# Xiaoming-Zhao/PointNav-VO

Hardware: AMD Instinct MI355X
Metric: RGB-D frame-pair VO inferences/s @341x192 (higher is better)
Workload: dtype f32

## Files before the change

### pointnav-vo_amd/csrc/conv_x3.hip

```cpp
#include <cmath>
#include <cstdio>
#include <cstdlib>
#include <cstring>

#include "pnvo_internal.h"

namespace pnvo {

typedef float f32x16 __attribute__((ext_vector_type(16)));
typedef float f32x4 __attribute__((ext_vector_type(4)));
typedef float f32x2 __attribute__((ext_vector_type(2)));
typedef __bf16 bf16x8 __attribute__((ext_vector_type(8)));
typedef __bf16 bf16x2 __attribute__((ext_vector_type(2)));
typedef _Float16 f16x8 __attribute__((ext_vector_type(8)));
typedef _Float16 f16x2 __attribute__((ext_vector_type(2)));
typedef unsigned u32x4 __attribute__((ext_vector_type(4)));

namespace {
__device__ __forceinline__ unsigned pack2(float a, float b) {
  const bf16x2 r = __builtin_convertvector(f32x2{a, b}, bf16x2);
  return __builtin_bit_cast(unsigned, r);
}
__device__ __forceinline__ unsigned pack2h(float a, float b) {
  const f16x2 r = __builtin_convertvector(f32x2{a, b}, f16x2);
  return __builtin_bit_cast(unsigned, r);
}
__device__ __forceinline__ float lo_f(unsigned u) { return __builtin_bit_cast(float, u << 16); }
__device__ __forceinline__ float hi_f(unsigned u) { return __builtin_bit_cast(float, u & 0xffff0000u); }
}

constexpr int x3_wpe(int mw, int nw, int np, bool dsf = false) {
  return dsf ? (mw * nw >= 6 ? 1 : (mw * nw >= 2 ? 2 : 3)) : ((np == 2 && mw * nw <= 2) ? 3 : 2);
}

template <int KS, int STRIDE, int MODE, int MW, int NW, int NP, bool DSF = false, bool W8 = false, bool KSW = false, bool M16 = false>
__global__ __launch_bounds__(W8 ? 512 : 256) __attribute__((amdgpu_waves_per_eu(W8 ? 2 : x3_wpe(MW, NW, NP, DSF), W8 ? 2 : x3_wpe(MW, NW, NP, DSF)))) void conv_x3_kernel(const ConvX3Args p) {
  constexpr int NTH = W8 ? 512 : 256, NWV = NTH / 64;
  constexpr int EMW = KSW ? 1 : MW;
  constexpr int NWT = M16 ? NW / 2 : NW;
  constexpr int TW = M16 ? (MW * NW + 3) / 4 : MW * NW;
  static_assert(!M16 || (NP == 2 && KS == 3 && STRIDE == 1 && !DSF && !KSW && NW % 2 == 0), "16x16x32 flavour: float16-piece 3x3 stride-1 convs, whole N-tiles");
  static_assert(!KSW || (NW == 1 && NP == 2 && KS == 3 && !DSF && !W8), "K split over the waves: float16-piece 3x3 convs, one N-tile");
  static_assert(!DSF || (KS == 3 && STRIDE == 2 && NP == 2 && (MODE == 0 || MODE == 2)), "the downsample rides on a float16-piece 3x3 stride-2 conv");
  extern __shared__ __attribute__((aligned(16))) unsigned char lds[];
  constexpr int PSTEP = KS == 1 ? STRIDE : 1;
  constexpr int CS = KS == 1 ? 1 : STRIDE;
  constexpr int PAD = KS / 2;
  const int lane = threadIdx.x & 63;
  const int wave = __builtin_amdgcn_readfirstlane(threadIdx.x >> 6);

  const int ntiles = p.B * p.tiles_r * p.tiles_c;
  const int chunk = (ntiles + 7) >> 3;
  int bid = (int)(blockIdx.x & 7) * chunk + (int)(blockIdx.x >> 3);
  if (bid >= ntiles) return;
  const int tci = bid % p.tiles_c;
  bid /= p.tiles_c;
  const int tri = bid % p.tiles_r;
  const int n = bid / p.tiles_r;
  const int r0 = tri * p.TR, c0 = tci * p.TC;
  const int hi0 = r0 * STRIDE - PAD, wi0 = c0 * STRIDE - PAD;
  const int mdl = (p.grp_end0 > 0 && n >= p.grp_end0) + (p.grp_end1 > 0 && n >= p.grp_end1);
  const unsigned short *g_wpk = mdl == 0 ? p.wpk : p.wpk_g[mdl - 1];
  const unsigned short *g_ds_wpk = mdl == 0 ? p.ds_wpk : p.ds_wpk_g[mdl - 1];
  const float g_oscale = mdl == 0 ? p.oscale : p.oscale_g[mdl - 1], g_ds_oscale = mdl == 0 ? p.ds_oscale : p.ds_oscale_g[mdl - 1];
  const float *g_gamma = mdl == 0 ? p.gn_gamma : p.gn_gamma_g[mdl - 1], *g_beta = mdl == 0 ? p.gn_beta : p.gn_beta_g[mdl - 1];
  const float *g_ds_gamma = mdl == 0 ? p.ds_gamma : p.ds_gamma_g[mdl - 1], *g_ds_beta = mdl == 0 ? p.ds_beta : p.ds_beta_g[mdl - 1];
  const int PR = p.PR, PC = p.PC, CK = p.CK;
  const int pitch = CK * 2 + 16;
  const int plane = PR * PC * pitch;
  const int npix = p.TR * p.TC;
  const int tab_off = KSW ? max(NP * plane, 4 * MW * 4096) : NP * plane;
  unsigned *qtab = reinterpret_cast<unsigned *>(lds + tab_off);
  unsigned *otab = qtab + p.MT * 32;
  for (int e = (int)threadIdx.x; e < p.MT * 32; e += NTH) {
    const int q = min(e, npix - 1);
    const int tr = q / p.TC, tc = q - tr * p.TC;
    qtab[e] = (unsigned)(((tr * CS) * PC + tc * CS) * pitch);
    const bool ok = e < npix && r0 + tr < p.Ho && c0 + tc < p.Wo;
    otab[e] = (unsigned)((tr * p.Wo + tc) * p.COUTP) | (ok ? 0u : 0x80000000u);
  }

  const int wn = p.wn;
  const int wave_m = wave / wn;
  const int wave_n = (wave & (wn - 1)) + (int)blockIdx.y * wn;
  const int ntt = p.COUTP >> 5, kct = p.CIN >> 4;

  f32x16 acc[MW][NW];
#pragma unroll
  for (int i = 0; i < MW; ++i)
#pragma unroll
    for (int j = 0; j < NW; ++j)
#pragma unroll
      for (int r = 0; r < 16; ++r) acc[i][j][r] = 0.f;
  f32x4 acc16[M16 ? MW : 1][M16 ? NW : 1];
  const int mt16 = (npix + 15) >> 4;
  const int m16_row = (mt16 + NWV / wn - 1) / (NWV / wn), m16_sub0 = wave_m * m16_row;
  const bool m16_last = m16_sub0 + MW <= mt16 && MW <= m16_row;
  if (M16) {
#pragma unroll
    for (int i = 0; i < MW; ++i)
#pragma unroll
      for (int j = 0; j < NW; ++j) acc16[M16 ? i : 0][M16 ? j : 0] = f32x4{0.f, 0.f, 0.f, 0.f};
  }
  f32x16 accd[DSF ? MW : 1][DSF ? NW : 1];
  if (DSF) {
#pragma unroll
    for (int i = 0; i < MW; ++i)
#pragma unroll
      for (int j = 0; j < NW; ++j)
#pragma unroll
        for (int r = 0; r < 16; ++r) accd[DSF ? i : 0][DSF ? j : 0][r] = 0.f;
  }

  float in_mul = 1.f, in_div = 1.f;
  const bool in_scaled = NP == 2 && p.in_absmax != nullptr;
  if (in_scaled) {
    unsigned mb = p.in_absmax[(threadIdx.x & 63) * 16];
#pragma unroll
    for (int d = 32; d >= 1; d >>= 1) mb = max(mb, (unsigned)__shfl_xor((int)mb, d));
    const int e = mb != 0u ? (int)((mb >> 23) & 0xffu) - 126 : 14;
    in_mul = __builtin_bit_cast(float, (unsigned)(14 - e + 127) << 23);
    in_div = __builtin_bit_cast(float, (unsigned)(e - 14 + 127) << 23);
  }
  const int G = CK >> 3;
  const int cg = threadIdx.x & (G - 1), pl = threadIdx.x / G, PS = NTH / G;
  const int dr = PS / PC, dc = PS - dr * PC;
  const int nppix = PR * PC;

  unsigned long long c_stage = 0, c_mm = 0, t_0 = __builtin_readcyclecounter(), r_0 = wall_clock64();
  for (int ck0 = 0; ck0 < p.CIN; ck0 += CK) {
    unsigned long long t_a = __builtin_readcyclecounter();
    if (ck0 > 0) __syncthreads();
    {
      f32x4 sc0, sc1, sh0, sh1, rs0, rs1, rt0, rt1;
      const bool res_ss = MODE == 2 && p.res_scale != nullptr;
      auto load_ss = [&]() {
        if (MODE >= 1) {
          const float *ps = p.in_scale + (long)n * p.CIN + ck0 + 8 * cg;
          const float *pt = p.in_shift + (long)n * p.CIN + ck0 + 8 * cg;
          sc0 = *reinterpret_cast<const f32x4 *>(ps);
          sc1 = *reinterpret_cast<const f32x4 *>(ps + 4);
          sh0 = *reinterpret_cast<const f32x4 *>(pt);
          sh1 = *reinterpret_cast<const f32x4 *>(pt + 4);
        }
        if (res_ss) {
          const float *ps = p.res_scale + (long)n * p.CIN + ck0 + 8 * cg;
          const float *pt = p.res_shift + (long)n * p.CIN + ck0 + 8 * cg;
          rs0 = *reinterpret_cast<const f32x4 *>(ps);
          rs1 = *reinterpret_cast<const f32x4 *>(ps + 4);
          rt0 = *reinterpret_cast<const f32x4 *>(pt);
          rt1 = *reinterpret_cast<const f32x4 *>(pt + 4);
        }
      };
      load_ss();
      int pr = pl / PC, pc = pl - pr * PC;
      const long img = ((long)n * p.H * p.W) * p.CIN + ck0 + 8 * cg;
      const float *xb = p.x + img;
      struct Round {
        f32x4 v[2][2], w[2][2];
        unsigned off[2];
        int gofs[2];
        bool ok[2], in[2], own[2];
      };
      auto fetch = [&](int pix, Round &r) {
#pragma unroll
        for (int k = 0; k < 2; ++k) {
          const int hi = hi0 + pr * PSTEP, wi = wi0 + pc * PSTEP;
          r.ok[k] = pix + k * PS < nppix;
          r.in[k] = r.ok[k] && hi >= 0 && hi < p.H && wi >= 0 && wi < p.W;
          r.off[k] = (unsigned)((pr * PC + pc) * pitch + 16 * cg);
          r.v[k][0] = r.v[k][1] = f32x4{0.f, 0.f, 0.f, 0.f};
          if (MODE >= 2) {
            r.own[k] = r.in[k] && p.xout != nullptr && blockIdx.y == 0 && pr >= PAD && pr < PAD + p.TR * CS && pc >= PAD && pc < PAD + p.TC * CS;
            r.gofs[k] = (hi * p.W + wi) * p.CIN;
          }
          if (r.in[k]) {
            const float *src = xb + ((long)hi * p.W + wi) * p.CIN;
            r.v[k][0] = *reinterpret_cast<const f32x4 *>(src);
            r.v[k][1] = *reinterpret_cast<const f32x4 *>(src + 4);
            if (MODE == 2) {
              const float *rsrc = p.res + img + ((long)hi * p.W + wi) * p.CIN;
              r.w[k][0] = *reinterpret_cast<const f32x4 *>(rsrc);
              r.w[k][1] = *reinterpret_cast<const f32x4 *>(rsrc + 4);
            }
          }
          pr += dr;
          pc += dc;
          if (pc >= PC) {
            pc -= PC;
            pr += 1;
          }
        }
      };
      auto split_store = [&](const Round &r) {
#pragma unroll
        for (int k = 0; k < 2; ++k) {
          if (!r.ok[k]) continue;
          float f[8];
#pragma unroll
          for (int e = 0; e < 8; ++e) {
            float t = r.v[k][e >> 2][e & 3];
            if (MODE == 1) {
              const f32x4 &sc = e < 4 ? sc0 : sc1, &sh = e < 4 ? sh0 : sh1;
              t = r.in[k] ? fmaxf(__builtin_fmaf(t, sc[e & 3], sh[e & 3]), 0.f) : 0.f;
            }
            if (MODE == 3) {
              const f32x4 &sc = e < 4 ? sc0 : sc1, &sh = e < 4 ? sh0 : sh1;
              int key = __builtin_bit_cast(int, t);
              key = key >= 0 ? key : key ^ 0x7fffffff;
              t = r.in[k] ? fmaxf(__builtin_fmaf(__builtin_bit_cast(float, key), __builtin_fabsf(sc[e & 3]), sh[e & 3]), 0.f) : 0.f;
            }
            if (MODE == 2) {
              const f32x4 &sc = e < 4 ? sc0 : sc1, &sh = e < 4 ? sh0 : sh1;
              float u = r.w[k][e >> 2][e & 3];
              if (res_ss) u = __builtin_fmaf(u, (e < 4 ? rs0 : rs1)[e & 3], (e < 4 ? rt0 : rt1)[e & 3]);
              t = r.in[k] ? fmaxf(__builtin_fmaf(t, sc[e & 3], sh[e & 3]) + u, 0.f) : 0.f;
            }
            f[e] = t;
          }
          if (MODE >= 2 && r.own[k]) {
            float *dst = p.xout + img + r.gofs[k];
            *reinterpret_cast<f32x4 *>(dst) = f32x4{f[0], f[1], f[2], f[3]};
            *reinterpret_cast<f32x4 *>(dst + 4) = f32x4{f[4], f[5], f[6], f[7]};
          }
          if (NP == 2) {
            if (in_scaled) {
#pragma unroll
              for (int e = 0; e < 8; ++e) f[e] *= in_mul;
            }
            u32x4 o0, o1;
#pragma unroll
            for (int e = 0; e < 4; ++e) {
              const float a = f[2 * e], b = f[2 * e + 1];
              const f16x2 h = __builtin_convertvector(f32x2{a, b}, f16x2);
              o0[e] = __builtin_bit_cast(unsigned, h);
              o1[e] = pack2h(a - (float)h[0], b - (float)h[1]);
            }
            *reinterpret_cast<u32x4 *>(lds + r.off[k]) = o0;
            *reinterpret_cast<u32x4 *>(lds + plane + r.off[k]) = o1;
            continue;
          }
          u32x4 o0, o1, o2;
#pragma unroll
          for (int e = 0; e < 4; ++e) {
            const float a = f[2 * e], b = f[2 * e + 1];
            const unsigned h = pack2(a, b);
            const float ra = a - lo_f(h), rb = b - hi_f(h);
            const unsigned m = pack2(ra, rb);
            o0[e] = h;
            o1[e] = m;
            o2[e] = pack2(ra - lo_f(m), rb - hi_f(m));
          }
          *reinterpret_cast<u32x4 *>(lds + r.off[k]) = o0;
          *reinterpret_cast<u32x4 *>(lds + plane + r.off[k]) = o1;
          *reinterpret_cast<u32x4 *>(lds + 2 * plane + r.off[k]) = o2;
        }
      };
      constexpr bool PIPE = !((MODE == 2 && (TW >= 6 || (M16 && !W8) || x3_wpe(MW, NW, NP) == 3 || DSF)) || (DSF && MW * NW == 4));
      if (TW <= 2 && !(MODE == 2 && (x3_wpe(MW, NW, NP) == 3 || DSF))) {
        for (int pix = pl; pix < nppix; pix += 6 * PS) {
          Round r0, r1, r2;
          fetch(pix, r0);
          fetch(pix + 2 * PS, r1);
          fetch(pix + 4 * PS, r2);
          split_store(r0);
          split_store(r1);
          split_store(r2);
        }
      } else if (PIPE) {
        Round cur, nxt;
        fetch(pl, cur);
        for (int pix = pl; pix < nppix; pix += 2 * PS) {
          const bool more = pix + 2 * PS < nppix;
          if (more) fetch(pix + 2 * PS, nxt);
          split_store(cur);
          if (more) cur = nxt;
        }
      } else {
        for (int pix = pl; pix < nppix; pix += 2 * PS) {
          Round cur;
          fetch(pix, cur);
          split_store(cur);
        }
      }
    }
    __syncthreads();
    unsigned long long t_b = __builtin_readcyclecounter();
    c_stage += t_b - t_a;

    if constexpr (M16) {
      unsigned aoff[MW];
#pragma unroll
      for (int i = 0; i < MW; ++i) {
        const int sub = min(m16_sub0 + i, mt16 - 1);
        aoff[i] = qtab[sub * 16 + (lane & 15)] + (unsigned)((lane >> 4) * 16);
      }
      const int kcc = CK >> 4, kcp = CK >> 5;
      const int nsteps = KS * KS * kcp;
      const unsigned kstep = (unsigned)ntt * (NP * 1024u);
      const char *wb_n = reinterpret_cast<const char *>(g_wpk) + (long)(ck0 >> 4) * kstep;
      unsigned toff_n = 0;
      int kc_n = 0, kw_n = 0;
      auto advance = [&]() {
        ++kc_n;
        toff_n += 64;
        wb_n += 2 * kstep;
        if (kc_n == kcp) {
          kc_n = 0;
          toff_n += (unsigned)(pitch - kcp * 64);
          wb_n += (long)(kct - kcc) * kstep;
          if (++kw_n == KS) {
            kw_n = 0;
            toff_n += (unsigned)((PC - KS) * pitch);
          }
        }
      };
      const int kg = lane >> 4;
      unsigned voff[NW];
#pragma unroll
      for (int j = 0; j < NW; ++j)
        voff[j] = (unsigned)min(wave_n * NWT + (j >> 1), ntt - 1) * (NP * 1024u) + (unsigned)(kg >> 1) * kstep +
                  (unsigned)((kg & 1) * 32 + 16 * (j & 1) + (lane & 15)) * 16u;
      auto loadA = [&](int i, u32x4 (*a)[MW]) {
#pragma unroll
        for (int pc = 0; pc < NP; ++pc) a[pc][i] = *reinterpret_cast<const u32x4 *>(lds + pc * plane + aoff[i] + toff_n);
      };
      auto loadB = [&](u32x4 (*b)[NW]) {
#pragma unroll
        for (int j = 0; j < NW; ++j)
#pragma unroll
          for (int pc = 0; pc < NP; ++pc) b[pc][j] = *reinterpret_cast<const u32x4 *>(wb_n + (size_t)voff[j] + pc * 1024);
      };
      auto step = [&](u32x4 (*a)[MW], const u32x4 (*b)[NW]) {
#pragma unroll
        for (int i = 0; i < MW; ++i) {
          if (i == MW - 1 && !m16_last) break;
          constexpr int TA[3] = {1, 0, 0}, TB[3] = {0, 1, 0};
#pragma unroll
          for (int jt = 0; jt < NWT; ++jt)
#pragma unroll
            for (int t = 0; t < 3; ++t)
#pragma unroll
              for (int j = 2 * jt; j < 2 * jt + 2; ++j)
                acc16[M16 ? i : 0][M16 ? j : 0] = __builtin_amdgcn_mfma_f32_16x16x32_f16(__builtin_bit_cast(f16x8, a[TA[t]][i]), __builtin_bit_cast(f16x8, b[TB[t]][M16 ? j : 0]),
                                                                                         acc16[M16 ? i : 0][M16 ? j : 0], 0, 0, 0);
          __builtin_amdgcn_sched_barrier(0);
          loadA(i, a);
          __builtin_amdgcn_sched_barrier(0);
        }
      };
      u32x4 a[NP][MW], b0[NP][NW], b1[NP][NW];
      loadB(b0);
#pragma unroll
      for (int i = 0; i < MW; ++i) loadA(i, a);
      advance();
#pragma unroll 1
      for (int s = 0; s < nsteps; s += 2) {
        loadB(b1);
        __builtin_amdgcn_sched_barrier(0);
        step(a, b0);
        if (s + 2 < nsteps) advance();
        if (s + 1 < nsteps) {
          loadB(b0);
          __builtin_amdgcn_sched_barrier(0);
          step(a, b1);
          if (s + 3 < nsteps) advance();
        }
      }
    } else {
    unsigned aoff[MW];
#pragma unroll
    for (int i = 0; i < MW; ++i) {
      const int mt = min(KSW ? i : wave_m * MW + i, p.MT - 1);
      aoff[i] = qtab[mt * 32 + (lane & 31)] + (unsigned)((lane >> 5) * 16);
    }
    const int kcc = CK >> 4;
    const int nsteps = KS * KS * kcc;
    const unsigned kstep = (unsigned)ntt * (NP * 1024u);
    const char *wb_n = reinterpret_cast<const char *>(g_wpk) + (long)(ck0 >> 4) * kstep;
    unsigned toff_n = 0;
    int kc_n = 0, kw_n = 0;
    auto advance = [&]() {
      ++kc_n;
      toff_n += 32;
      wb_n += kstep;
      if (kc_n == kcc) {
        kc_n = 0;
        toff_n += (unsigned)(pitch - kcc * 32);
        wb_n += (long)(kct - kcc) * kstep;
        if (++kw_n == KS) {
          kw_n = 0;
          toff_n += (unsigned)((PC - KS) * pitch);
        }
      }
    };
    constexpr bool RING = NP == 2 && KS == 3 && MW * NW <= 2;
    const char *wb_b = wb_n;
    int kc_b = 0;
    auto advanceB = [&]() {
      wb_b += kstep;
      if (++kc_b == kcc) {
        kc_b = 0;
        wb_b += (long)(kct - kcc) * kstep;
      }
    };
    unsigned voff[NW];
#pragma unroll
    for (int j = 0; j < NW; ++j) voff[j] = (unsigned)min(wave_n * NW + j, ntt - 1) * (NP * 1024u) + (unsigned)lane * 16u;
    auto loadBr = [&](u32x4 (*b)[NW]) {
#pragma unroll
      for (int j = 0; j < NW; ++j)
#pragma unroll
        for (int pc = 0; pc < NP; ++pc) b[pc][j] = *reinterpret_cast<const u32x4 *>(wb_b + (size_t)voff[j] + pc * 1024);
    };
    auto loadA = [&](int i, u32x4 (*a)[MW]) {
#pragma unroll
      for (int pc = 0; pc < NP; ++pc) a[pc][i] = *reinterpret_cast<const u32x4 *>(lds + pc * plane + aoff[i] + toff_n);
    };
    auto loadB = [&](u32x4 (*b)[NW]) {
#pragma unroll
      for (int j = 0; j < NW; ++j)
#pragma unroll
        for (int pc = 0; pc < NP; ++pc) b[pc][j] = *reinterpret_cast<const u32x4 *>(wb_n + (size_t)voff[j] + pc * 1024);
    };
    auto step = [&](u32x4 (*a)[MW], const u32x4 (*b)[NW]) {
#pragma unroll
      for (int i = 0; i < MW; ++i) {
#pragma unroll
        for (int j = 0; j < NW; ++j) {
          if (NP == 2) {
            constexpr int TA[3] = {1, 0, 0}, TB[3] = {0, 1, 0};
#pragma unroll
            for (int t = 0; t < 3; ++t)
              acc[i][j] = __builtin_amdgcn_mfma_f32_32x32x16_f16(__builtin_bit_cast(f16x8, a[TA[t]][i]),
                                                                 __builtin_bit_cast(f16x8, b[TB[t]][j]), acc[i][j], 0, 0, 0);
          } else {
            constexpr int TA[6] = {1, 2, 0, 1, 0, 0}, TB[6] = {1, 0, 2, 0, 1, 0};
#pragma unroll
            for (int t = 0; t < 6; ++t)
              acc[i][j] = __builtin_amdgcn_mfma_f32_32x32x16_bf16(__builtin_bit_cast(bf16x8, a[TA[t]][i]),
                                                                  __builtin_bit_cast(bf16x8, b[TB[t]][j]), acc[i][j], 0, 0, 0);
          }
        }
        __builtin_amdgcn_sched_barrier(0);
        loadA(i, a);
        __builtin_amdgcn_sched_barrier(0);
      }
    };
    u32x4 a[NP][MW], b0[NP][NW], b1[NP][NW];
    u32x4 bd0[DSF ? NP : 1][NW], bd1[DSF ? NP : 1][NW];
    auto loadBd = [&](u32x4 (*b)[NW], int kc) {
      const char *wd = reinterpret_cast<const char *>(g_ds_wpk) + (long)((ck0 >> 4) + kc) * kstep;
#pragma unroll
      for (int j = 0; j < NW; ++j)
#pragma unroll
        for (int pc = 0; pc < NP; ++pc) b[pc][j] = *reinterpret_cast<const u32x4 *>(wd + (size_t)voff[j] + pc * 1024);
    };
    if constexpr (KSW) {
      const int s0 = (wave * nsteps) >> 2, s1 = ((wave + 1) * nsteps) >> 2;
      {
        const int tap = s0 / kcc, kc = s0 - tap * kcc, kh = tap / KS, kw = tap - kh * KS;
        kc_n = kc;
        kw_n = kw;
        toff_n = (unsigned)((kh * PC + kw) * pitch + kc * 32);
        wb_n += ((long)tap * kct + kc) * kstep;
        kc_b = kc;
        wb_b = wb_n;
      }
      u32x4 br[3][NP][NW];
      int fb = s0;
      auto fetchB = [&](u32x4 (*bq)[NW]) {
        loadBr(bq);
        if (++fb < s1) advanceB();
      };
      fetchB(br[0]);
      fetchB(br[1]);
#pragma unroll
      for (int i = 0; i < MW; ++i) loadA(i, a);
      if (s0 + 1 < s1) advance();
#pragma unroll 1
      for (int s = s0; s < s1; s += 3) {
#pragma unroll
        for (int u = 0; u < 3; ++u) {
          if (s + u >= s1) break;
          fetchB(br[(u + 2) % 3]);
          __builtin_amdgcn_sched_barrier(0);
          step(a, br[u]);
          if (s + u + 2 < s1) advance();
        }
      }
    } else {
    if (DSF) loadBd(bd0, 0);
    loadB(b0);
#pragma unroll
    for (int i = 0; i < MW; ++i) loadA(i, a);
    advance();
    if (RING) {
      constexpr int R = MW * NW <= 2 ? 6 : 3;
      u32x4 br[R][NP][NW];
#pragma unroll
      for (int pc = 0; pc < NP; ++pc)
#pragma unroll
        for (int j = 0; j < NW; ++j) br[0][pc][j] = b0[pc][j];
#pragma unroll
      for (int q = 1; q < R - 1; ++q) {
        advanceB();
        loadBr(br[q]);
      }
      advanceB();
      constexpr bool A2 = MW * NW <= 2 && !(MODE == 2 && MW * NW == 2 && !DSF) && !(MODE == 2 && DSF && MW * NW == 1);
      u32x4 a1[A2 ? NP : 1][MW];
      if (A2) {
#pragma unroll
        for (int i = 0; i < MW; ++i) loadA(i, a1);
        advance();
      }
#pragma unroll 1
      for (int s = 0; s < nsteps; s += R) {
#pragma unroll
        for (int u = 0; u < R; ++u) {
          loadBr(br[(u + R - 1) % R]);
          if (s + u + R < nsteps) advanceB();
          __builtin_amdgcn_sched_barrier(0);
          if (A2) {
            step((u & 1) ? a1 : a, br[u]);
            if (s + u + 3 < nsteps) advance();
          } else {
            step(a, br[u]);
            if (s + u + 2 < nsteps) advance();
          }
        }
      }
    } else {
#pragma unroll 1
      for (int s = 0; s < nsteps; s += 2) {
        const bool more = s + 2 < nsteps;
        loadB(b1);
        __builtin_amdgcn_sched_barrier(0);
        step(a, b0);
        if (more) advance();
        loadB(b0);
        __builtin_amdgcn_sched_barrier(0);
        step(a, b1);
        if (more) advance();
      }
    }
    }
    if constexpr (DSF) {
      const unsigned tc0 = (unsigned)((PC + 1) * pitch);
      u32x4 ad[NP][MW];
      auto loadAd = [&](int kc) {
#pragma unroll
        for (int i = 0; i < MW; ++i)
#pragma unroll
          for (int pc = 0; pc < NP; ++pc) ad[pc][i] = *reinterpret_cast<const u32x4 *>(lds + pc * plane + aoff[i] + tc0 + (unsigned)kc * 32u);
      };
      auto mm = [&](const u32x4 (*bd)[NW]) {
        constexpr int TA[3] = {1, 0, 0}, TB[3] = {0, 1, 0};
#pragma unroll
        for (int i = 0; i < MW; ++i)
#pragma unroll
          for (int j = 0; j < NW; ++j)
// ... 989 lines not shown
```

Measured before the change: 115,300.

## Add deep-batched buffer-load stager for residual-add tail in K-split convs

For mode-2 (residual add + ReLU) float16-piece 3x3 convs with K split over waves and MW==3, staging now uses a separate path. It issues up to seven pixels' buffer loads of x and the residual before converting and splitting any of them into LDS. Buffer resources with out-of-range offsets replace the per-pixel branches for bounds and ownership, and the scale/shift loads are moved after the first fetch. The aim is more memory-level parallelism in the input staging, paid for with higher register pressure from the many in-flight pixels.

Result: slower. 113,500 (-1.6%).

```diff
diff --git a/pointnav-vo_amd/csrc/conv_x3.hip b/pointnav-vo_amd/csrc/conv_x3.hip
--- a/pointnav-vo_amd/csrc/conv_x3.hip
+++ b/pointnav-vo_amd/csrc/conv_x3.hip
@@ -39,6 +39,10 @@
   constexpr int EMW = KSW ? 1 : MW;
   constexpr int NWT = M16 ? NW / 2 : NW;
   constexpr int TW = M16 ? (MW * NW + 3) / 4 : MW * NW;
+  constexpr bool TAIL_WINS = NP == 2 && KS == 3 && KSW && MW == 3;
+  constexpr int TAIL_FIT = (256 - (DSF ? 32 : 16) * MW * NW - 76) / 17;
+  constexpr int TAILP = MODE != 2 || !TAIL_WINS ? 0 : (TAIL_FIT > 7 ? 7 : TAIL_FIT);
+  static_assert(TAILP == 0 || TAILP >= 3, "fewer than three pixels in flight: the predicated stager's round has two");
   static_assert(!M16 || (NP == 2 && KS == 3 && STRIDE == 1 && !DSF && !KSW && NW % 2 == 0), "16x16x32 flavour: float16-piece 3x3 stride-1 convs, whole N-tiles");
   static_assert(!KSW || (NW == 1 && NP == 2 && KS == 3 && !DSF && !W8), "K split over the waves: float16-piece 3x3 convs, one N-tile");
   static_assert(!DSF || (KS == 3 && STRIDE == 2 && NP == 2 && (MODE == 0 || MODE == 2)), "the downsample rides on a float16-piece 3x3 stride-2 conv");
@@ -123,7 +127,7 @@
     in_div = __builtin_bit_cast(float, (unsigned)(e - 14 + 127) << 23);
   }
   const int G = CK >> 3;
-  const int cg = threadIdx.x & (G - 1), pl = threadIdx.x / G, PS = NTH / G;
+  const int cg0 = threadIdx.x & (G - 1), pl = threadIdx.x / G, PS = NTH / G;
   const int dr = PS / PC, dc = PS - dr * PC;
   const int nppix = PR * PC;
 
@@ -134,6 +138,8 @@
     {
       f32x4 sc0, sc1, sh0, sh1, rs0, rs1, rt0, rt1;
       const bool res_ss = MODE == 2 && p.res_scale != nullptr;
+      int cg = cg0;
+      if (TAILP > 0) asm volatile("" : "+v"(cg));
       auto load_ss = [&]() {
         if (MODE >= 1) {
           const float *ps = p.in_scale + (long)n * p.CIN + ck0 + 8 * cg;
@@ -143,16 +149,16 @@
           sh0 = *reinterpret_cast<const f32x4 *>(pt);
           sh1 = *reinterpret_cast<const f32x4 *>(pt + 4);
         }
-        if (res_ss) {
-          const float *ps = p.res_scale + (long)n * p.CIN + ck0 + 8 * cg;
-          const float *pt = p.res_shift + (long)n * p.CIN + ck0 + 8 * cg;
+        if (MODE == 2 && (res_ss || TAILP > 0)) {
+          const float *ps = (res_ss ? p.res_scale : p.in_scale) + (long)n * p.CIN + ck0 + 8 * cg;
+          const float *pt = (res_ss ? p.res_shift : p.in_shift) + (long)n * p.CIN + ck0 + 8 * cg;
           rs0 = *reinterpret_cast<const f32x4 *>(ps);
           rs1 = *reinterpret_cast<const f32x4 *>(ps + 4);
           rt0 = *reinterpret_cast<const f32x4 *>(pt);
           rt1 = *reinterpret_cast<const f32x4 *>(pt + 4);
         }
       };
-      load_ss();
+      if (TAILP == 0) load_ss();
       int pr = pl / PC, pc = pl - pr * PC;
       const long img = ((long)n * p.H * p.W) * p.CIN + ck0 + 8 * cg;
       const float *xb = p.x + img;
@@ -256,8 +262,97 @@
           *reinterpret_cast<u32x4 *>(lds + 2 * plane + r.off[k]) = o2;
         }
       };
+      struct Tail {
+        f32x4 v[2], w[2];
+        unsigned code;
+      };
+      __amdgpu_buffer_rsrc_t dsc_x, dsc_r, dsc_o;
+      if (TAILP > 0) {
+        const unsigned pbytes = (unsigned)(p.H * p.W * p.CIN - ck0) * 4u;
+        dsc_x = __builtin_amdgcn_make_buffer_rsrc((void *)(p.x + ((long)n * p.H * p.W) * p.CIN + ck0), 0, pbytes, 0x00020000);
+        dsc_r = __builtin_amdgcn_make_buffer_rsrc((void *)(p.res + ((long)n * p.H * p.W) * p.CIN + ck0), 0, pbytes, 0x00020000);
+        const bool wr = p.xout != nullptr && blockIdx.y == 0;
+        dsc_o = __builtin_amdgcn_make_buffer_rsrc((void *)((wr ? p.xout : const_cast<float *>(p.x)) + ((long)n * p.H * p.W) * p.CIN + ck0), 0, wr ? pbytes : 0u, 0x00020000);
+      }
+      auto fetch_tail = [&](int pix, Tail &r) {
+        const int hi = hi0 + pr * PSTEP, wi = wi0 + pc * PSTEP;
+        const bool in = (pix < nppix) & ((unsigned)hi < (unsigned)p.H) & ((unsigned)wi < (unsigned)p.W);
+        const bool own = ((unsigned)(pr - PAD) < (unsigned)(p.TR * CS)) & ((unsigned)(pc - PAD) < (unsigned)(p.TC * CS));
+        const unsigned o = in ? (unsigned)(((hi * p.W + wi) * p.CIN + 8 * cg) * 4) : 0x80000000u;
+        r.code = o | ((in & own) ? 1u : 0u);
+        r.v[0] = __builtin_bit_cast(f32x4, __builtin_amdgcn_raw_buffer_load_b128(dsc_x, o, 0, 0));
+        r.v[1] = __builtin_bit_cast(f32x4, __builtin_amdgcn_raw_buffer_load_b128(dsc_x, o + 16u, 0, 0));
+        r.w[0] = __builtin_bit_cast(f32x4, __builtin_amdgcn_raw_buffer_load_b128(dsc_r, o, 0, 0));
+        r.w[1] = __builtin_bit_cast(f32x4, __builtin_amdgcn_raw_buffer_load_b128(dsc_r, o + 16u, 0, 0));
+        const int wrap = pc + dc >= PC ? 1 : 0;
+        pr += dr + wrap;
+        pc += dc - wrap * PC;
+      };
+      auto to_lds = [&](float *f, unsigned off) {
+        if (NP == 2) {
+          if (in_scaled) {
+#pragma unroll
+            for (int e = 0; e < 8; ++e) f[e] *= in_mul;
+          }
+          u32x4 o0, o1;
+#pragma unroll
+          for (int e = 0; e < 4; ++e) {
+            const float a = f[2 * e], b = f[2 * e + 1];
+            const f16x2 h = __builtin_convertvector(f32x2{a, b}, f16x2);
+            o0[e] = __builtin_bit_cast(unsigned, h);
+            o1[e] = pack2h(a - (float)h[0], b - (float)h[1]);
+          }
+          *reinterpret_cast<u32x4 *>(lds + off) = o0;
+          *reinterpret_cast<u32x4 *>(lds + plane + off) = o1;
+          return;
+        }
+        u32x4 o0, o1, o2;
+#pragma unroll
+        for (int e = 0; e < 4; ++e) {
+          const float a = f[2 * e], b = f[2 * e + 1];
+          const unsigned h = pack2(a, b);
+          const float ra = a - lo_f(h), rb = b - hi_f(h);
+          const unsigned m = pack2(ra, rb);
+          o0[e] = h;
+          o1[e] = m;
+          o2[e] = pack2(ra - lo_f(m), rb - hi_f(m));
+        }
+        *reinterpret_cast<u32x4 *>(lds + off) = o0;
+        *reinterpret_cast<u32x4 *>(lds + plane + off) = o1;
+        *reinterpret_cast<u32x4 *>(lds + 2 * plane + off) = o2;
+      };
+      auto split_tail = [&](int q, const Tail &r) {
+        asm volatile("" : "+v"(q));
+        if (q >= nppix) return;
+        const unsigned keep = (int)r.code >= 0 ? 0xffffffffu : 0u;
+        float f[8];
+#pragma unroll
+        for (int e = 0; e < 8; ++e) {
+          const f32x4 &sc = e < 4 ? sc0 : sc1, &sh = e < 4 ? sh0 : sh1;
+          float u = r.w[e >> 2][e & 3];
+          if (res_ss) u = __builtin_fmaf(u, (e < 4 ? rs0 : rs1)[e & 3], (e < 4 ? rt0 : rt1)[e & 3]);
+          const float t = fmaxf(__builtin_fmaf(r.v[e >> 2][e & 3], sc[e & 3], sh[e & 3]) + u, 0.f);
+          f[e] = __builtin_bit_cast(float, __builtin_bit_cast(unsigned, t) & keep);
+        }
+        const unsigned so = (r.code & 0x80000001u) == 1u ? r.code ^ 1u : 0x80000000u;
+        __builtin_amdgcn_raw_buffer_store_b128(__builtin_bit_cast(u32x4, f32x4{f[0], f[1], f[2], f[3]}), dsc_o, so, 0, 0);
+        __builtin_amdgcn_raw_buffer_store_b128(__builtin_bit_cast(u32x4, f32x4{f[4], f[5], f[6], f[7]}), dsc_o, so + 16u, 0, 0);
+        to_lds(f, (unsigned)(q * pitch + 16 * cg));
+      };
       constexpr bool PIPE = !((MODE == 2 && (TW >= 6 || (M16 && !W8) || x3_wpe(MW, NW, NP) == 3 || DSF)) || (DSF && MW * NW == 4));
-      if (TW <= 2 && !(MODE == 2 && (x3_wpe(MW, NW, NP) == 3 || DSF))) {
+      if constexpr (TAILP > 0) {
+        asm volatile("" : "+v"(pr), "+v"(pc));
+        for (int pix = pl; pix < nppix; pix += TAILP * PS) {
+          Tail r[TAILP];
+#pragma unroll
+          for (int j = 0; j < TAILP; ++j) {
+            fetch_tail(pix + j * PS, r[j]);
+            if (j == 0) load_ss();
+          }
+#pragma unroll
+          for (int j = 0; j < TAILP; ++j) split_tail(pix + j * PS, r[j]);
+        }
+      } else if (TW <= 2 && !(MODE == 2 && (x3_wpe(MW, NW, NP) == 3 || DSF))) {
         for (int pix = pl; pix < nppix; pix += 6 * PS) {
           Round r0, r1, r2;
           fetch(pix, r0);
```
